# zhongzisha/multi_frame_super_resolution

Hardware: AMD Instinct MI355X
Metric: Mpix/s end-to-end (N-frame burst -> x2 SR) (higher is better)
Workload: dtype f32

## Files before the change

include/mfsr.h:

```cpp
#ifndef MFSR_H
#define MFSR_H

#include <stddef.h>
#include <stdint.h>

#ifdef __cplusplus
extern "C" {
#endif

#define MFSR_VERSION 100
#define MFSR_MAX_FUSE_GROUP 4

typedef void* mfsr_stream_t;

typedef struct { float x, y; } mfsr_float2;
typedef struct { float x, y, z; } mfsr_float3;
typedef struct { float x, y, z, w; } mfsr_float4;

typedef struct {
    const void* ptr;
    int32_t pitch;
    int32_t width;
    int32_t height;
} mfsr_tex2d;
// ... 162 lines not shown
                             int tileCount, mfsr_stream_t stream);
int mfsr_addRoundedPreShift(const mfsr_float2* preShift, int prePitch, mfsr_float2* found, int foundPitch, int countX,
                            int countY, mfsr_stream_t stream);
int mfsr_scaleFlow(mfsr_float2* flow, int pitch, int width, int height, float factor, mfsr_stream_t stream);
int mfsr_float3ToFloat4(const mfsr_float3* in, int inPitch, mfsr_float4* out, int outPitch, int width, int height,
                        mfsr_stream_t stream);
int mfsr_resampleFloat3(const mfsr_float3* in, int inPitch, int inW, int inH, mfsr_float3* out, int outPitch, int outW,
                        int outH, float u0, float u1, float v0, float v1, mfsr_stream_t stream);
int mfsr_quantize(const mfsr_float3* in, int inPitch, uint16_t* out16, uint8_t* out8, int width, int height,
                  float maxOut, mfsr_stream_t stream);
int mfsr_fill_f32(float* dst, size_t count, float value, mfsr_stream_t stream);
int mfsr_prepareFrameFused(const uint16_t* dataIn, mfsr_float3* halfOut, int halfPitch, float maxVal, int dimX, int dimY,
                           float* pyr0, int pyr0Pitch, float* pyr1, int pyr1Pitch, const float* taps, int ntaps,
                           mfsr_stream_t stream);
int mfsr_zeroRing_f32x4(mfsr_float4* img, int pitch, int width, int height, mfsr_stream_t stream);
int mfsr_set_accumulate_fast_exp(int enable);

int mfsr_trackTilesFused(const float* refImg, const float* movedImg, const mfsr_float2* preShift, int preShiftPitch,
                         mfsr_float2* coordinates, int coordinatesPitch, int imgWidth, int imgHeight, int imgPitch,
                         int maxShift, int tileSize, int tileCountX, int tileCountY, float threshold,
                         const float* refSquaredSums, mfsr_stream_t stream);
int mfsr_tileSquaredSums(const float* refImg, float* outValues, int imgWidth, int imgHeight, int imgPitch, int maxShift,
                         int tileSize, int tileCountX, int tileCountY, mfsr_stream_t stream);
int mfsr_lucasKanadeIterationFused(const mfsr_float2* shiftsIn, mfsr_float2* shiftsOut, int pitchShift,
                                   const float* refImg, const float* movedImg, int pitchImg, int width, int height,
                                   int halfWindowSize, float minDet, float outScale, mfsr_stream_t stream);
int mfsr_robustnessMaskFused(const mfsr_float3* rawImgRef, const mfsr_float3* rawImgMoved, mfsr_float4* robustnessMask,
                             mfsr_tex2d texUV, int imgWidth, int imgHeight, int imgPitch, int maskPitch, float alpha, float beta,
                             float thresholdM, mfsr_stream_t stream);
int mfsr_set_robustness_fast(int enable);
int mfsr_structureTensorFused(const float* img, int imgPitch, mfsr_float3* outImg, int outPitch, int width, int height,
                              mfsr_stream_t stream);
int mfsr_deBayerFused(const uint16_t* raw, mfsr_float3* outImage, int strideOut, int width, int height,
                      mfsr_float3 blackPoint, mfsr_float3 scale, mfsr_stream_t stream);
int mfsr_finishFused(const mfsr_float3* finalImg, const mfsr_float3* weight, int imgPitch, const mfsr_float3* fallback,
                     int fbPitch, int fbW, int fbH, float u0, float u1, float v0, float v1, mfsr_float3* outImg,
                     int outPitch, uint16_t* out16, int width, int height, float threshold, int applyGamma,
                     float maxOut, mfsr_stream_t stream);

typedef struct {
    float shiftX, shiftY;
    float rotation;
    float cosRotation, sinRotation;
    int32_t angleIndex, tx, ty, level;
    int32_t reserved[3];
} mfsr_prealign;
size_t mfsr_preAlign_pyramid_bytes(int width, int height);
size_t mfsr_preAlign_workspace_bytes(float maxAngleDeg);
int mfsr_preAlign_init(void* workspace, float maxAngleDeg, mfsr_stream_t stream);
int mfsr_preAlignPyramid(const float* img, int width, int height, int pitch, void* pyramid, mfsr_stream_t stream);
int mfsr_preAlign(const void* refPyramid, const void* movedPyramid, int width, int height, float maxAngleDeg,
                  void* workspace, mfsr_prealign* result, mfsr_stream_t stream);
int mfsr_preAlign_identity(mfsr_prealign* result, mfsr_stream_t stream);
int mfsr_trackTilesFusedBase(const float* refImg, const float* movedImg, const mfsr_float2* preShift, int preShiftPitch,
                             mfsr_float2* coordinates, int coordinatesPitch, int imgWidth, int imgHeight, int imgPitch,
// ... 249 lines not shown
```

multi_frame_super_resolution_amd/csrc/debayer.hip:

```cpp
#include <cstring>
#include "common.hpp"

static int g_cfa[4] = {MFSR_RED, MFSR_GREEN, MFSR_GREEN, MFSR_BLUE};

int mfsr_cfa_packed() { return (g_cfa[0] & 0xff) | ((g_cfa[1] & 0xff) << 8) | ((g_cfa[2] & 0xff) << 16) | ((g_cfa[3] & 0xff) << 24); }

extern "C" int mfsr_set_cfa_pattern(const int32_t pattern[4])
{
    MFSR_REQUIRE(pattern != nullptr);
    for (int i = 0; i < 4; i++) MFSR_REQUIRE(pattern[i] >= 0 && pattern[i] <= MFSR_WHITE);
    for (int i = 0; i < 4; i++) g_cfa[i] = pattern[i];
    return MFSR_OK;
}

extern "C" int mfsr_get_cfa_pattern(int32_t pattern[4])
{
    MFSR_REQUIRE(pattern != nullptr);
    for (int i = 0; i < 4; i++) pattern[i] = g_cfa[i];
    return MFSR_OK;
}

__global__ void __launch_bounds__(256) k_deBayersSubSample3(const uint16_t* __restrict__ dataIn, pix3* __restrict__ imgOut,
                                                           float maxVal, int dimX, int dimY, int strideOut, int cfa)
{
// ... 324 lines not shown
                g = RAWC(x, y, 1);
            } else if (thisPixel == MFSR_RED || thisPixel == MFSR_BLUE) {
                const int c = (thisPixel == MFSR_RED) ? 0 : 2;
                const float p = RAWC(x, y, c);
                const float xMinus2 = RAWC(x - 2, y, c), xMinus1 = RAWC(x - 1, y, 1), xPlus1 = RAWC(x + 1, y, 1),
                            xPlus2 = RAWC(x + 2, y, c);
                const float yMinus2 = RAWC(x, y - 2, c), yMinus1 = RAWC(x, y - 1, 1), yPlus1 = RAWC(x, y + 1, 1),
                            yPlus2 = RAWC(x, y + 2, c);
                const float gradientX = 0.5f * fabsf(xPlus1 - xMinus1);
                const float gradientY = 0.5f * fabsf(yPlus1 - yMinus1);
                const float laplaceX = 0.25f * fabsf(2.0f * p - xMinus2 - xPlus2);
                const float laplaceY = 0.25f * fabsf(2.0f * p - yMinus2 - yPlus2);
                const float interpolX = 0.125f * (-xMinus2 + 4.0f * xMinus1 + 2.0f * p + 4.0f * xPlus1 - xPlus2);
                const float interpolY = 0.125f * (-yMinus2 + 4.0f * yMinus1 + 2.0f * p + 4.0f * yPlus1 - yPlus2);
                const float weight = (gradientY + laplaceY) / (gradientX + gradientY + laplaceX + laplaceY + 0.000000001f);
                g = weight * interpolX + (1.0f - weight) * interpolY;
            }
#undef RAWC
        }
        s_g[ly][lx] = g;
    }
    __syncthreads();
    const int x = x0 + threadIdx.x, y = y0 + threadIdx.y;
    if (x >= width - 2 || x < 2 || y >= height - 2 || y < 2) return;
    auto GREENF = [&](int xx, int yy) { return s_g[yy - y0 + 1][xx - x0 + 1]; };
#define RAWR(xx, yy) ((RAWF(xx, yy) - L.bp[0]) * L.sc[0])
#define RAWB(xx, yy) ((RAWF(xx, yy) - L.bp[2]) * L.sc[2])
    const int thisPixel = cfa_at(cfa, y, x);
    const int thisRow = cfa_at(cfa, y, x + 1);
    const float g = GREENF(x, y);
    float r = 0.0f, b = 0.0f;
    if (thisPixel == MFSR_GREEN) {
        if (thisRow == MFSR_RED) {
            r = g + 0.5f * ((RAWR(x - 1, y) - GREENF(x - 1, y)) + (RAWR(x + 1, y) - GREENF(x + 1, y)));
            b = g + 0.5f * ((RAWB(x, y - 1) - GREENF(x, y - 1)) + (RAWB(x, y + 1) - GREENF(x, y + 1)));
        } else {
            b = g + 0.5f * ((RAWB(x - 1, y) - GREENF(x - 1, y)) + (RAWB(x + 1, y) - GREENF(x + 1, y)));
            r = g + 0.5f * ((RAWR(x, y - 1) - GREENF(x, y - 1)) + (RAWR(x, y + 1) - GREENF(x, y + 1)));
        }
    } else if (thisPixel == MFSR_RED) {
        r = RAWR(x, y);
        b = g + 0.25f * ((((RAWB(x - 1, y - 1) - GREENF(x - 1, y - 1)) + (RAWB(x + 1, y - 1) - GREENF(x + 1, y - 1))) +
                          (RAWB(x + 1, y + 1) - GREENF(x + 1, y + 1))) +
                         (RAWB(x - 1, y + 1) - GREENF(x - 1, y + 1)));
    } else if (thisPixel == MFSR_BLUE) {
        b = RAWB(x, y);
        r = g + 0.25f * ((((RAWR(x - 1, y - 1) - GREENF(x - 1, y - 1)) + (RAWR(x + 1, y - 1) - GREENF(x + 1, y - 1))) +
// ... 20 lines not shown
```

multi_frame_super_resolution_amd/csrc/glue.hip:

```cpp
#include <cmath>
#include <cstring>

#include "common.hpp"

extern "C" const char* mfsr_error_string(int code)
{
    switch (code) {
        case MFSR_OK: return "success";
        case MFSR_E_INVALID: return "invalid argument";
        case MFSR_E_UNSUPPORTED: return "unsupported parameter";
        case MFSR_E_NODEVICE: return "no HIP device";
        case MFSR_E_WORKSPACE: return "workspace too small";
        case -5: return "multi-GPU transport failed (mfsr_dist: RCCL error, or a peer of a local group failed / timed out)";
        default: break;
    }
    if (code > 0) return hipGetErrorString((hipError_t)code);
    return "unknown error";
}

extern "C" int mfsr_version(void) { return MFSR_VERSION; }

extern "C" int mfsr_device_count(void)
{
    int n = 0;
    if (hipGetDeviceCount(&n) != hipSuccess) {
        (void)hipGetLastError();
// ... 479 lines not shown
    t0 += s_t[ly][lx - 1] * 8.0f;
    t0 -= s_t[ly][lx - 2];
    t0 /= 12.0f;
    const float dx = t0;
    t0 = s_t[ly + 2][lx];
    t0 -= s_t[ly + 1][lx] * 8.0f;
    t0 += s_t[ly - 1][lx] * 8.0f;
    t0 -= s_t[ly - 2][lx];
    t0 /= 12.0f;
    const float dy = t0;
    pix3 val = {dx * dx, dy * dy, dx * dy};
    row_ptr(outImg, outPitch, y)[x] = val;
}

extern "C" int mfsr_structureTensorFused(const float* img, int imgPitch, mfsr_float3* outImg, int outPitch, int width,
                                         int height, mfsr_stream_t stream)
{
    MFSR_REQUIRE(img && outImg && width >= 4 && height >= 4 && (long long)imgPitch >= 4LL * width &&
                 (long long)outPitch >= 12LL * width && (imgPitch & 3) == 0 && (outPitch & 3) == 0);
    dim3 block(ST_TX, ST_TY), grid(mfsr_cdiv(width, ST_TX), mfsr_cdiv(height, ST_TY));
    hipLaunchKernelGGL(k_structureTensorFused, grid, block, 0, mfsr_s(stream), img, imgPitch, (pix3*)outImg, outPitch,
                       width, height);
    return mfsr_launch_status("structureTensorFused");
}

__device__ __forceinline__ float apply_weight_f(float inout, float val, float w, float threshold)
{
    if (w < threshold) {
        val += inout;
        w += 1;
    }
    inout = 0;
    if (w != 0) inout = val / w;
    return inout;
}

__device__ __forceinline__ float gamma_f(float v)
{
    if (isnan(v)) v = 0;
    v = fmaxf(fminf(v, 1.0f), 0.0f);
    if (v <= 0.0031308f) return 12.92f * v;
    return (1.0f + 0.055f) * powf(v, 1.0f / 2.4f) - 0.055f;
}

__global__ void __launch_bounds__(256)
    k_finishFused(const pix3* __restrict__ finalImg, const pix3* __restrict__ weight, int imgPitch,
// ... 147 lines not shown
```

multi_frame_super_resolution_amd/csrc/optical_flow.hip:

```cpp
#include "common.hpp"
#include "lk_math.hpp"

__global__ void __launch_bounds__(256)
    k_Warping(int width, int height, int stride, mfsr_tex2d texUV, float* __restrict__ out, mfsr_tex2d texToWarp)
{
    const int ix = threadIdx.x + blockIdx.x * blockDim.x;
    const int iy = threadIdx.y + blockIdx.y * blockDim.y;
    if (ix >= width || iy >= height) return;
    const float2 shift = tex2<ADDR_CLAMP>(texUV, ((float)ix + 0.5f) / (float)width, ((float)iy + 0.5f) / (float)height);
    const float x = ((float)ix + 0.5f + shift.x) / (float)width;
    const float y = ((float)iy + 0.5f + shift.y) / (float)height;
    row_ptr(out, stride, iy)[ix] = tex1<ADDR_MIRROR>(texToWarp, x, y);
}

extern "C" int mfsr_WarpingKernel(int width, int height, int stride, mfsr_tex2d texUV, float* out, mfsr_tex2d texToWarp,
                                  mfsr_stream_t stream)
{
    MFSR_REQUIRE(out && width > 0 && height > 0 && (long long)stride >= 4LL * width && (stride & 3) == 0);
    MFSR_REQUIRE(mfsr_tex_ok(texUV, 8) && ((uintptr_t)texUV.ptr & 7) == 0 && (texUV.pitch & 7) == 0);
    MFSR_REQUIRE(mfsr_tex_ok(texToWarp, 4) && (texToWarp.pitch & 3) == 0);
    dim3 block(64, 4), grid(mfsr_cdiv(width, 64), mfsr_cdiv(height, 4));
    hipLaunchKernelGGL(k_Warping, grid, block, 0, mfsr_s(stream), width, height, stride, texUV, out, texToWarp);
    return mfsr_launch_status("WarpingKernel");
}
// ... 57 lines not shown
    shift.x += cf * patchCenterX - sf * patchCenterY - patchCenterX;
    shift.y += sf * patchCenterX + cf * patchCenterY - patchCenterY;
    const float2 shiftPatch =
        tex2<ADDR_CLAMP>(texShift, ((float)pxX + 0.5f) / (float)imgWidth, ((float)pxY + 0.5f) / (float)imgHeight);
    shift.x += shiftPatch.x;
    shift.y += shiftPatch.y;
    row_ptr(outImg, imgPitch, pxY)[pxX] = shift;
}

extern "C" int mfsr_CreateFlowFieldFromTilesBase(mfsr_float2* outImg, mfsr_tex2d texObjShiftXY, int imgWidth, int imgHeight,
                                                 int imgPitch, const mfsr_prealign* base, mfsr_stream_t stream)
{
    MFSR_REQUIRE(outImg && base && imgWidth > 0 && imgHeight > 0);
    MFSR_REQUIRE((long long)imgPitch >= 8LL * imgWidth && (imgPitch & 7) == 0 && ((uintptr_t)outImg & 7) == 0);
    MFSR_REQUIRE(mfsr_tex_ok(texObjShiftXY, 8) && ((uintptr_t)texObjShiftXY.ptr & 7) == 0 && (texObjShiftXY.pitch & 7) == 0);
    dim3 block(64, 4), grid(mfsr_cdiv(imgWidth, 64), mfsr_cdiv(imgHeight, 4));
    hipLaunchKernelGGL(k_CreateFlowFieldFromTilesBase, grid, block, 0, mfsr_s(stream), (float2*)outImg, texObjShiftXY, imgWidth,
                       imgHeight, imgPitch, base);
    return mfsr_launch_status("CreateFlowFieldFromTilesBase");
}

__device__ __forceinline__ float deriv5(const mfsr_tex2d& t, float x, float y, float dx, float dy)
{
    float t0 = tex1<ADDR_MIRROR>(t, x + 2.0f * dx, y + 2.0f * dy);
    t0 -= tex1<ADDR_MIRROR>(t, x + 1.0f * dx, y + 1.0f * dy) * 8.0f;
    t0 += tex1<ADDR_MIRROR>(t, x - 1.0f * dx, y - 1.0f * dy) * 8.0f;
    t0 -= tex1<ADDR_MIRROR>(t, x - 2.0f * dx, y - 2.0f * dy);
    t0 /= 12.0f;
    return t0;
}

__global__ void __launch_bounds__(256) k_ComputeDerivatives(int width, int height, int stride, float* __restrict__ Ix,
                                                           float* __restrict__ Iy, float* __restrict__ Iz,
                                                           mfsr_tex2d texSource, mfsr_tex2d texTarget)
{
    const int ix = threadIdx.x + blockIdx.x * blockDim.x;
    const int iy = threadIdx.y + blockIdx.y * blockDim.y;
    if (ix >= width || iy >= height) return;
    const float dx = 1.0f / (float)width;
    const float dy = 1.0f / (float)height;
    const float x = ((float)ix + 0.5f) * dx;
    const float y = ((float)iy + 0.5f) * dy;
    float t0 = deriv5(texSource, x, y, dx, 0.0f);
    float t1 = deriv5(texTarget, x, y, dx, 0.0f);
    row_ptr(Ix, stride, iy)[ix] = (t0 + t1) * 0.5f;
    row_ptr(Iz, stride, iy)[ix] = tex1<ADDR_MIRROR>(texSource, x, y) - tex1<ADDR_MIRROR>(texTarget, x, y);
    t0 = deriv5(texSource, x, y, 0.0f, dy);
    t1 = deriv5(texTarget, x, y, 0.0f, dy);
    row_ptr(Iy, stride, iy)[ix] = (t0 + t1) * 0.5f;
}

extern "C" int mfsr_ComputeDerivativesKernel(int width, int height, int stride, float* Ix, float* Iy, float* Iz,
// ... 105 lines not shown
```

multi_frame_super_resolution_amd/csrc/pipeline.cpp:

```cpp
#include <hip/hip_runtime.h>

#include <cmath>
#include <cstdio>
#include <cstring>
#include <new>
#include <utility>
#include <vector>

#include "common.hpp"
#include "raw_stage.hpp"

namespace {

constexpr int kMaxLevels = 4;
constexpr int kMaxTimedLaunches = 4096;
constexpr int kRing = 2 * MFSR_MAX_FUSE_GROUP;
constexpr int kMaxUploadRing = 32;

inline size_t align_up(size_t v, size_t a) { return (v + a - 1) / a * a; }

struct Img {
    void* ptr = nullptr;
    int pitch = 0;
    int w = 0, h = 0;
// ... 587 lines not shown
    const int nl = ilog2(L.maxFactor) + 1;
    for (int i = 1; i < nl; i++)
        TRY(mfsr_downsample2x((const float*)pyr[i - 1].ptr, pyr[i - 1].pitch, (float*)pyr[i].ptr, pyr[i].pitch, pyr[i].w,
                              pyr[i].h, stream));
    return MFSR_OK;
}

static int set_reference_impl(mfsr_burst* b, const uint16_t* rawRef, int hrRow0, int hrRow1, mfsr_stream_t stream)
{
    MFSR_REQUIRE(b && rawRef);
    TRY(flush_pending(b, stream, false));
    const mfsr_config& c = b->cfg;
    Layout& L = b->L;
    MFSR_REQUIRE(hrRow0 >= 0 && hrRow1 > hrRow0 && hrRow1 <= L.hrH);
    MFSR_REQUIRE(!b->winNext.on || (hrRow0 == 0 && hrRow1 == L.hrH));
    b->win = b->winNext;
    if (b->win.on) {
        hrRow0 = b->win.y0;
        hrRow1 = b->win.y0 + b->win.h;
    }
    const bool whole = (hrRow0 == 0 && hrRow1 == L.hrH) || !c.fused;
    TRY(wait_uploads(b, stream));
    if (!b->refPrepared) TRY(prepare_frame(b, rawRef, L.refHalf, L.refPyr, stream));
    if (c.fused)
        for (int l = 0; l < c.levels; l++) {
            const Img& ref = L.refPyr[ilog2(c.levelFactor[l])];
            TRY(mfsr_tileSquaredSums((const float*)ref.ptr, L.refSq[l], ref.w, ref.h, ref.pitch, c.maxShift[l], c.tileSize[l],
                                     L.tcx[l], L.tcy[l], stream));
        }

    if (c.preAlign) {
        TRY(mfsr_preAlign_init(L.preWork, c.preAlignMaxAngle, stream));
        if (!b->refPrepared)
            TRY(mfsr_preAlignPyramid((const float*)L.refPyr[0].ptr, L.tw, L.th, L.refPyr[0].pitch, L.preRefPyr, stream));
    }

    static const bool refOverlap = [] {
        const char* e = getenv("MFSR_REF_OVERLAP");
        return !(e && e[0] == '0');
    }();
    mfsr_stream_t es = stream;
    b->refOnFuse = false;
    if (refOverlap && b->fuseStream && c.fused) {
        MFSR_HIP_TRY(hipEventRecord(b->evRefStart, mfsr_s(stream)));
        MFSR_HIP_TRY(hipStreamWaitEvent(b->fuseStream, b->evRefStart, 0));
        es = (mfsr_stream_t)b->fuseStream;
    }
    {
        int f0 = 0, f1 = L.th;
        if (!whole) {
            const int per = L.hrH / L.th, halo = b->ntensorTaps / 2 + 1;
            f0 = hrRow0 / per - 1 - halo;
            f1 = (hrRow1 + per - 1) / per + 1 + halo;
            f0 = f0 < 0 ? 0 : f0;
            f1 = f1 > L.th ? L.th : f1;
        }
        const int fr = f1 - f0;
        Img& ix = L.Ix;
        Img& iy = L.Iy;
        auto rows = [&](const Img& im) { return (char*)im.ptr + (size_t)f0 * im.pitch; };
        TRY(mfsr_ComputeDerivatives2Rows(L.tw, L.th, ix.pitch, (float*)ix.ptr, (float*)iy.ptr, as_tex(L.refPyr[0]), f0, fr, es));
        TRY(mfsr_ComputeStructureTensor((const float*)rows(ix), (const float*)rows(iy), (mfsr_float3*)rows(L.tensor), L.tw, fr, ix.pitch,
                                        L.tensor.pitch, es));
        TRY(mfsr_separableFilter((const float*)rows(L.tensor), L.tensor.pitch, (float*)rows(L.tensorTmp), (float*)rows(L.tensorSm),
                                 L.tensorSm.pitch, L.tw, fr, 3, b->tensorTaps, b->ntensorTaps, es));
        TRY(mfsr_ComputeKernelParam((mfsr_float3*)rows(L.tensorSm), L.tw, fr, L.tensorSm.pitch, c.Dth, c.Dtr, c.kDetail, c.kDenoise,
                                    c.kStretch, c.kShrink, es));
        TRY(mfsr_float3ToFloat4((const mfsr_float3*)rows(L.tensorSm), L.tensorSm.pitch, (mfsr_float4*)rows(L.kparam4), L.kparam4.pitch,
                                L.tw, fr, es));
    }

    const mfsr_float3 bp = {c.black[0], c.black[1], c.black[2]};
    const mfsr_float3 sc = {1.0f / c.white[0], 1.0f / c.white[1], 1.0f / c.white[2]};
    int r0 = 0, r1 = L.H;
    if (!whole) {
        r0 = (hrRow0 / c.scale - 8) & ~1;
        r1 = ((hrRow1 + c.scale - 1) / c.scale + 8 + 1) & ~1;
        r0 = r0 < 0 ? 0 : r0;
        r1 = r1 > L.H ? L.H : r1;
    }
    char* fb = (char*)L.fallback.ptr + (size_t)r0 * L.fallback.pitch;
    MFSR_HIP_TRY(hipMemsetAsync(fb, 0, (size_t)L.fallback.pitch * (r1 - r0), mfsr_s(es)));
    if (c.fused) {
        TRY(mfsr_deBayerFused(rawRef + (size_t)r0 * L.W, (mfsr_float3*)fb, L.fallback.pitch, L.W, r1 - r0, bp, sc, es));
        if (es != stream) {
            MFSR_HIP_TRY(hipEventRecord(b->evRefDone, b->fuseStream));
            b->refOnFuse = true;
        }
    } else {
        TRY(mfsr_u16ToFloat(rawRef, (float*)L.rawf.ptr, L.rawf.pitch, L.W, L.H, 1.0f, stream));
        TRY(mfsr_deBayerGreenKernel(L.W, L.H, (const float*)L.rawf.ptr, L.rawf.pitch, (mfsr_float3*)L.fallback.ptr,
                                    L.fallback.pitch, bp, sc, stream));
        TRY(mfsr_deBayerRedBlueKernel(L.W, L.H, (const float*)L.rawf.ptr, L.rawf.pitch, (mfsr_float3*)L.fallback.ptr,
                                      L.fallback.pitch, bp, sc, stream));
    }
    b->haveRef = true;
    b->refStale = false;
    b->framesSinceRef = 0;
    b->holdLastGroup = false;
    return MFSR_OK;
}

extern "C" int mfsr_burst_set_reference(mfsr_burst* b, const uint16_t* rawRef, mfsr_stream_t stream)
{
    MFSR_REQUIRE(b != nullptr);
    return set_reference_impl(b, rawRef, 0, b->L.hrH, stream);
}

extern "C" int mfsr_burst_set_reference_rows(mfsr_burst* b, const uint16_t* rawRef, int hrRow0, int hrRow1, mfsr_stream_t stream)
{
    MFSR_REQUIRE(b != nullptr);
    return set_reference_impl(b, rawRef, hrRow0, hrRow1, stream);
// ... 1845 lines not shown
```

multi_frame_super_resolution_amd/csrc/tile_tracker.hip:

```cpp
#include <cfloat>

#include <cstdlib>

#include <cstring>
#include "common.hpp"

__device__ __forceinline__ float wave_sum(float v)
{
#pragma unroll
    for (int off = 32; off >= 1; off >>= 1) v += __shfl_xor(v, off, 64);
    return v;
}
__device__ __forceinline__ float wave_max(float v)
{
#pragma unroll
    for (int off = 32; off >= 1; off >>= 1) v = fmaxf(v, __shfl_xor(v, off, 64));
    return v;
}
__device__ __forceinline__ void wave_argmin(float& v, int& idx)
{
#pragma unroll
    for (int off = 32; off >= 1; off >>= 1) {
        const float ov = __shfl_xor(v, off, 64);
        const int oi = __shfl_xor(idx, off, 64);
        const bool take = (ov < v) || (ov == v && oi < idx);
        v = take ? ov : v;
        idx = take ? oi : idx;
    }
// ... 406 lines not shown
                                                               int imgOutPitch)
{
    const int pxX = blockIdx.x * blockDim.x + threadIdx.x;
    const int pxY = blockIdx.y * blockDim.y + threadIdx.y;
    if (pxX >= imgWidth || pxY >= imgHeight) return;
    const float dx = row_ptr(imgDx, imgDxDyPitch, pxY)[pxX];
    const float dy = row_ptr(imgDy, imgDxDyPitch, pxY)[pxX];
    pix3 val = {dx * dx, dy * dy, dx * dy};
    row_ptr(outImg, imgOutPitch, pxY)[pxX] = val;
}

extern "C" int mfsr_ComputeStructureTensor(const float* imgDx, const float* imgDy, mfsr_float3* outImg, int imgWidth,
                                           int imgHeight, int imgDxDyPitch, int imgOutPitch, mfsr_stream_t stream)
{
    MFSR_REQUIRE(imgDx && imgDy && outImg && imgWidth > 0 && imgHeight > 0);
    MFSR_REQUIRE((long long)imgDxDyPitch >= 4LL * imgWidth && (long long)imgOutPitch >= 12LL * imgWidth);
    MFSR_REQUIRE((imgDxDyPitch & 3) == 0 && (imgOutPitch & 3) == 0);
    dim3 block(64, 4), grid(mfsr_cdiv(imgWidth, 64), mfsr_cdiv(imgHeight, 4));
    hipLaunchKernelGGL(k_ComputeStructureTensor, grid, block, 0, mfsr_s(stream), imgDx, imgDy, (pix3*)outImg, imgWidth,
                       imgHeight, imgDxDyPitch, imgOutPitch);
    return mfsr_launch_status("ComputeStructureTensor");
}

__device__ __forceinline__ pix3 kernel_param(pix3 grad, float Dth, float Dtr, float kDetail, float kDenoise,
                                             float kStretch, float kShrink)
{
    const float a11 = grad.x, a22 = grad.y, a12 = grad.z;
    const float help = sqrtf((a22 - a11) * (a22 - a11) + 4.0f * a12 * a12);
    float c = 2.0f * a12;
    float s = a22 - a11 + help;
    const float norm = sqrtf(c * c + s * s);
    if (norm > 0) {
        c /= norm;
        s /= norm;
    } else {
        c = 1;
        s = 0;
    }
    const float lam1 = (a11 + a22 + help) / 2.0f;
    const float lam2 = (a11 + a22 - help) / 2.0f;
    const float A = 1 + sqrtf((lam1 - lam2) * (lam1 - lam2) / ((lam1 + lam2) * (lam1 + lam2)));
    float D = 1 - sqrtf(lam1) / Dtr + Dth;
    D = fmaxf(fminf(1.0f, D), 0.0f);
    const float k1h = kDetail * kStretch * A;
    const float k2h = kDetail / kShrink * A;
    float k1 = ((1.0f - D) * k1h + D * kDetail * kDenoise);
    float k2 = ((1.0f - D) * k2h + D * kDetail * kDenoise);
    k1 *= k1;
    k2 *= k2;
    const float x2 = c, y2 = s, x1 = s, y1 = -c;
    const float b11 = k1 * x1 * x1 + x2 * x2 * k2;
    const float b12 = k1 * x1 * y1 + x2 * y2 * k2;
    const float b22 = k1 * y1 * y1 + y2 * y2 * k2;
    const float det = b11 * b22 - b12 * b12 + 0.0000000001f;
    pix3 kernel = {b22 / det, b11 / det, -b12 / det};
    return kernel;
}

__global__ void __launch_bounds__(256) k_ComputeKernelParam(pix3* __restrict__ kernelImg, int imgWidth, int imgHeight,
                                                           int imgOutPitch, float Dth, float Dtr, float kDetail,
                                                           float kDenoise, float kStretch, float kShrink)
{
    const int pxX = blockIdx.x * blockDim.x + threadIdx.x;
    const int pxY = blockIdx.y * blockDim.y + threadIdx.y;
    if (pxX >= imgWidth || pxY >= imgHeight) return;
    pix3* p = row_ptr(kernelImg, imgOutPitch, pxY) + pxX;
    *p = kernel_param(*p, Dth, Dtr, kDetail, kDenoise, kStretch, kShrink);
}

extern "C" int mfsr_ComputeKernelParam(mfsr_float3* kernelImg, int imgWidth, int imgHeight, int imgOutPitch, float Dth,
                                       float Dtr, float kDetail, float kDenoise, float kStretch, float kShrink,
                                       mfsr_stream_t stream)
{
    MFSR_REQUIRE(kernelImg && imgWidth > 0 && imgHeight > 0 && (long long)imgOutPitch >= 12LL * imgWidth);
    MFSR_REQUIRE((imgOutPitch & 3) == 0);
    dim3 block(64, 4), grid(mfsr_cdiv(imgWidth, 64), mfsr_cdiv(imgHeight, 4));
    hipLaunchKernelGGL(k_ComputeKernelParam, grid, block, 0, mfsr_s(stream), (pix3*)kernelImg, imgWidth, imgHeight,
                       imgOutPitch, Dth, Dtr, kDetail, kDenoise, kStretch, kShrink);
    return mfsr_launch_status("ComputeKernelParam");
}

// ... 476 lines not shown
        for (int y = 0; y < T; y++) box += rq[y * R];
        const float sq = refSq[min(tile0 + sl, tileCount - 1)];
        slot_dist(sl)[cand] = sq + box - 2 * cc;
    }
    __syncthreads();

    const int wave = tid >> 6, lane = tid & 63;
    if (wave < TPW && tile0 + wave < tileCount) {
        const int tileIdx = tile0 + wave;
        float minVal, maxVal;
        int minIdx;
        wave_min_argmin_max(slot_dist(wave), R * R, lane, minVal, minIdx, maxVal);
        if (lane == 0) {
            const int tileIdxY = tileIdx / tileCountX, tileIdxX = tileIdx - tileIdxY * tileCountX;
            const float2 pre = s_pre[wave];
            float2 coord = subpixel_minimum(slot_dist(wave), S, minVal, minIdx, maxVal, threshold);
            coord.x = roundf(pre.x) + coord.x;
            coord.y = roundf(pre.y) + coord.y;
            row_ptr(coordinates, coordinatesPitch, tileIdxY)[tileIdxX] = coord;
        }
    }
}

__global__ void __launch_bounds__(64)
    k_tileSquaredSums(const float* __restrict__ refImg, float* __restrict__ out, int imgWidth, int imgHeight, int imgPitch,
                      int maxShift, int tileSize, int tileCountX, int tileCountY)
{
    extern __shared__ __attribute__((aligned(16))) float s_mem[];
    const int T = tileSize, S = maxShift;
    const int tileIdx = blockIdx.x;
    const int tileIdxY = tileIdx / tileCountX, tileIdxX = tileIdx - tileIdxY * tileCountX;
    const float2 zero2 = make_float2(0.0f, 0.0f);
    for (int i = threadIdx.x; i < T * T; i += 64) {
        const int y = i / T, x = i - y * T;
        s_mem[i] = tile_fetch(refImg, imgWidth, imgHeight, imgPitch, T, tileIdxX, tileIdxY, x + S, y + S, zero2, zero2, 0.0f);
    }
    __syncthreads();
    if (threadIdx.x == 0) {
        float a = 0;
        for (int i = 0; i < T * T; i++) a += s_mem[i] * s_mem[i];
        out[tileIdx] = a;
    }
}

extern "C" int mfsr_tileSquaredSums(const float* refImg, float* outValues, int imgWidth, int imgHeight, int imgPitch,
                                    int maxShift, int tileSize, int tileCountX, int tileCountY, mfsr_stream_t stream)
{
    MFSR_REQUIRE(refImg && outValues && imgWidth > 0 && imgHeight > 0);
    MFSR_REQUIRE((long long)imgPitch >= 4LL * imgWidth && (imgPitch & 3) == 0);
    MFSR_REQUIRE(maxShift >= 1 && maxShift <= 15 && tileSize >= 4 && tileSize <= 128 && tileCountX > 0 && tileCountY > 0);
    hipLaunchKernelGGL(k_tileSquaredSums, dim3(tileCountX * tileCountY), dim3(64), sizeof(float) * tileSize * tileSize,
                       mfsr_s(stream), refImg, outValues, imgWidth, imgHeight, imgPitch, maxShift, tileSize, tileCountX,
                       tileCountY);
    return mfsr_launch_status("tileSquaredSums");
}

static int track_tiles_fused_impl(const float* refImg, const float* movedImg, const mfsr_float2* preShift, int preShiftPitch,
                                  mfsr_float2* coordinates, int coordinatesPitch, int imgWidth, int imgHeight, int imgPitch,
                                  int maxShift, int tileSize, int tileCountX, int tileCountY, float threshold,
                                  const float* refSquaredSums, const mfsr_prealign* base, float baseInvScale,
                                  const mfsr_float2* coarse, int coarsePitch, int4 up, int upOldTile, mfsr_stream_t stream,
                                  int nFrames = 1, const MfsrBatch* batch = nullptr)
{
    MfsrBatch bt;
    if (batch)
        bt = *batch;
    else
        memset(&bt, 0, sizeof(bt));
    MFSR_REQUIRE(refImg && movedImg && coordinates && imgWidth > 0 && imgHeight > 0);
    MFSR_REQUIRE((long long)imgPitch >= 4LL * imgWidth && (imgPitch & 3) == 0);
    MFSR_REQUIRE(maxShift >= 1 && maxShift <= 15 && tileSize >= 4 && tileSize <= 128 && tileCountX > 0 && tileCountY > 0);
    MFSR_REQUIRE((long long)coordinatesPitch >= 8LL * tileCountX && (coordinatesPitch & 7) == 0 &&
                 ((uintptr_t)coordinates & 7) == 0);
    if (preShift)
        MFSR_REQUIRE((long long)preShiftPitch >= 8LL * tileCountX && (preShiftPitch & 7) == 0 && ((uintptr_t)preShift & 7) == 0);
    static const bool fast = [] {
        const char* e = getenv("MFSR_TRK_FAST");
// ... 115 lines not shown
```

Before: 22350.

## Fuse kernel-parameter chain into one tiled kernel and batch squared-sum levels

Replaces the five-launch chain of derivatives, structure tensor, separable smoothing, kernel parameter and float3-to-float4 conversion with one tiled kernel. It stages the image, derivatives and horizontally filtered tensor in LDS, so the intermediates never go to global memory. It also merges the per-level tileSquaredSums launches into a single launch that indexes levels by block. The fallback memset is dropped by having the fused debayer write zeros on its border. The cost is a large LDS footprint that may limit occupancy, plus recomputing halo derivatives in every tile.

```diff
diff --git a/include/mfsr.h b/include/mfsr.h
--- a/include/mfsr.h
+++ b/include/mfsr.h
@@ -208,6 +208,12 @@
                          const float* refSquaredSums, mfsr_stream_t stream);
 int mfsr_tileSquaredSums(const float* refImg, float* outValues, int imgWidth, int imgHeight, int imgPitch, int maxShift,
                          int tileSize, int tileCountX, int tileCountY, mfsr_stream_t stream);
+typedef struct {
+    const float* refImg;
+    float* outValues;
+    int imgWidth, imgHeight, imgPitch, maxShift, tileSize, tileCountX, tileCountY, reserved;
+} mfsr_sqsum_level;
+int mfsr_tileSquaredSumsLevels(int nLevels, const mfsr_sqsum_level* levels, mfsr_stream_t stream);
 int mfsr_lucasKanadeIterationFused(const mfsr_float2* shiftsIn, mfsr_float2* shiftsOut, int pitchShift,
                                    const float* refImg, const float* movedImg, int pitchImg, int width, int height,
                                    int halfWindowSize, float minDet, float outScale, mfsr_stream_t stream);
@@ -217,6 +223,14 @@
 int mfsr_set_robustness_fast(int enable);
 int mfsr_structureTensorFused(const float* img, int imgPitch, mfsr_float3* outImg, int outPitch, int width, int height,
                               mfsr_stream_t stream);
+int mfsr_kernelParamChain(mfsr_tex2d tex, float* Ix, float* Iy, int derivPitch, mfsr_float3* tensor, mfsr_float3* tensorTmp,
+                          mfsr_float3* tensorSm, int tensorPitch, mfsr_float4* kparam4, int kparamPitch, int row0, int rows,
+                          const float* taps, int ntaps, float Dth, float Dtr, float kDetail, float kDenoise, float kStretch,
+                          float kShrink, mfsr_stream_t stream);
+int mfsr_kernelParamFused(mfsr_tex2d tex, float* Ix, float* Iy, int derivPitch, mfsr_float3* tensor, mfsr_float3* tensorTmp,
+                          mfsr_float3* tensorSm, int tensorPitch, mfsr_float4* kparam4, int kparamPitch, int row0, int rows,
+                          const float* taps, int ntaps, float Dth, float Dtr, float kDetail, float kDenoise, float kStretch,
+                          float kShrink, mfsr_stream_t stream);
 int mfsr_deBayerFused(const uint16_t* raw, mfsr_float3* outImage, int strideOut, int width, int height,
                       mfsr_float3 blackPoint, mfsr_float3 scale, mfsr_stream_t stream);
 int mfsr_finishFused(const mfsr_float3* finalImg, const mfsr_float3* weight, int imgPitch, const mfsr_float3* fallback,
diff --git a/multi_frame_super_resolution_amd/csrc/debayer.hip b/multi_frame_super_resolution_amd/csrc/debayer.hip
--- a/multi_frame_super_resolution_amd/csrc/debayer.hip
+++ b/multi_frame_super_resolution_amd/csrc/debayer.hip
@@ -370,7 +370,12 @@
     }
     __syncthreads();
     const int x = x0 + threadIdx.x, y = y0 + threadIdx.y;
-    if (x >= width - 2 || x < 2 || y >= height - 2 || y < 2) return;
+    if (x >= width || y >= height) return;
+    if (x >= width - 2 || x < 2 || y >= height - 2 || y < 2) {
+        const pix3 z = {0.0f, 0.0f, 0.0f};
+        row_ptr(outImage, strideOut, y)[x] = z;
+        return;
+    }
     auto GREENF = [&](int xx, int yy) { return s_g[yy - y0 + 1][xx - x0 + 1]; };
 #define RAWR(xx, yy) ((RAWF(xx, yy) - L.bp[0]) * L.sc[0])
 #define RAWB(xx, yy) ((RAWF(xx, yy) - L.bp[2]) * L.sc[2])
diff --git a/multi_frame_super_resolution_amd/csrc/glue.hip b/multi_frame_super_resolution_amd/csrc/glue.hip
--- a/multi_frame_super_resolution_amd/csrc/glue.hip
+++ b/multi_frame_super_resolution_amd/csrc/glue.hip
@@ -2,6 +2,7 @@
 #include <cstring>
 
 #include "common.hpp"
+#include "kernel_field.hpp"
 
 extern "C" const char* mfsr_error_string(int code)
 {
@@ -527,6 +528,155 @@
     hipLaunchKernelGGL(k_structureTensorFused, grid, block, 0, mfsr_s(stream), img, imgPitch, (pix3*)outImg, outPitch,
                        width, height);
     return mfsr_launch_status("structureTensorFused");
+}
+
+#define KPF_TX 64
+#define KPF_TY 16
+#define KPF_MAXC0 8
+struct KpfTaps {
+    float t[2 * KPF_MAXC0 + 1];
+    int n;
+};
+struct KpfShape {
+    float Dth, Dtr, kDetail, kDenoise, kStretch, kShrink;
+};
+
+__global__ void __launch_bounds__(256) k_kernelParamFused(mfsr_tex2d tex, float4* __restrict__ kparam4, int outPitch, int row0,
+                                                         int rows, KpfTaps taps, KpfShape ks)
+{
+    extern __shared__ __attribute__((aligned(16))) float s_kpf[];
+    const int c0 = taps.n / 2;
+    const int DW = KPF_TX + 2 * c0, DH = KPF_TY + 2 * c0;
+    const int SW = DW + 6, SH = DH + 6;
+    float* sImg = s_kpf;
+    float* sIx = sImg + SW * SH;
+    float* sIy = sIx + DW * DH;
+    float* sXX = sIy + DW * DH;
+    float* sYY = sXX + KPF_TX * DH;
+    float* sXY = sYY + KPF_TX * DH;
+    const int W = tex.width, H = tex.height;
+    const float* __restrict__ img = (const float*)tex.ptr;
+    const int tid = threadIdx.y * 64 + threadIdx.x;
+    const int x0 = blockIdx.x * KPF_TX, y0 = row0 + blockIdx.y * KPF_TY, yEnd = row0 + rows;
+    const int ox = x0 - c0 - 3, oy = y0 - c0 - 3;
+
+    {
+        const int stepY = 256 / SW, stepX = 256 - stepY * SW;
+        int ly = tid / SW, lx = tid - ly * SW;
+        while (ly < SH) {
+            sImg[ly * SW + lx] = row_ptr(img, tex.pitch, clampi(oy + ly, 0, H - 1))[clampi(ox + lx, 0, W - 1)];
+            lx += stepX;
+            ly += stepY;
+            if (lx >= SW) {
+                lx -= SW;
+                ly++;
+            }
+        }
+    }
+    __syncthreads();
+    {
+        auto texel = [&](int i, int j) {
+            const int li = i - ox, lj = j - oy;
+            if ((unsigned)li < (unsigned)SW && (unsigned)lj < (unsigned)SH) return sImg[lj * SW + li];
+            return row_ptr(img, tex.pitch, j)[i];
+        };
+        auto fetch = [&](float u, float v) { return tex1_with<ADDR_MIRROR>(W, H, u, v, texel); };
+        const float dx = 1.0f / (float)W;
+        const float dy = 1.0f / (float)H;
+        const int stepY = 256 / DW, stepX = 256 - stepY * DW;
+        int ly = tid / DW, lx = tid - ly * DW;
+        while (ly < DH) {
+            const int gx = clampi(x0 + lx - c0, 0, W - 1), gy = clampi(y0 + ly - c0, row0, yEnd - 1);
+            const float x = ((float)gx + 0.5f) * dx;
+            const float y = ((float)gy + 0.5f) * dy;
+            sIx[ly * DW + lx] = deriv5_with(fetch, x, y, dx, 0.0f);
+            sIy[ly * DW + lx] = deriv5_with(fetch, x, y, 0.0f, dy);
+            lx += stepX;
+            ly += stepY;
+            if (lx >= DW) {
+                lx -= DW;
+                ly++;
+            }
+        }
+    }
+    __syncthreads();
+    for (int i = tid; i < KPF_TX * DH; i += 256) {
+        const int ly = i >> 6, lx = i & 63;
+        float sxx = 0, syy = 0, sxy = 0;
+        for (int t = 0; t < taps.n; t++) {
+            const float gx = sIx[ly * DW + lx + t], gy = sIy[ly * DW + lx + t], w = taps.t[t];
+            sxx = __fadd_rn(sxx, __fmul_rn(w, __fmul_rn(gx, gx)));
+            syy = __fadd_rn(syy, __fmul_rn(w, __fmul_rn(gy, gy)));
+            sxy = __fadd_rn(sxy, __fmul_rn(w, __fmul_rn(gx, gy)));
+        }
+        sXX[i] = sxx;
+        sYY[i] = syy;
+        sXY[i] = sxy;
+    }
+    __syncthreads();
+    const int lx = threadIdx.x, gx = x0 + lx;
+#pragma unroll
+    for (int r = 0; r < KPF_TY / 4; r++) {
+        const int ly = threadIdx.y + 4 * r, gy = y0 + ly;
+        if (gx >= W || gy >= yEnd) continue;
+        pix3 s = {0.0f, 0.0f, 0.0f};
+        for (int t = 0; t < taps.n; t++) {
+            const float w = taps.t[t];
+            s.x = __fadd_rn(s.x, __fmul_rn(w, sXX[(ly + t) * KPF_TX + lx]));
+            s.y = __fadd_rn(s.y, __fmul_rn(w, sYY[(ly + t) * KPF_TX + lx]));
+            s.z = __fadd_rn(s.z, __fmul_rn(w, sXY[(ly + t) * KPF_TX + lx]));
+        }
+        const pix3 p = kernel_param(s, ks.Dth, ks.Dtr, ks.kDetail, ks.kDenoise, ks.kStretch, ks.kShrink);
+        row_ptr(kparam4, outPitch, gy)[gx] = make_float4(p.x, p.y, p.z, 0.0f);
+    }
+}
+
+extern "C" int mfsr_kernelParamChain(mfsr_tex2d tex, float* Ix, float* Iy, int derivPitch, mfsr_float3* tensor, mfsr_float3* tensorTmp,
+                                     mfsr_float3* tensorSm, int tensorPitch, mfsr_float4* kparam4, int kparamPitch, int row0, int rows,
+                                     const float* taps, int ntaps, float Dth, float Dtr, float kDetail, float kDenoise, float kStretch,
+                                     float kShrink, mfsr_stream_t stream)
+{
+    MFSR_REQUIRE(Ix && Iy && tensor && tensorTmp && tensorSm && kparam4 && mfsr_tex_ok(tex, 4));
+    MFSR_REQUIRE(row0 >= 0 && rows > 0 && row0 + rows <= tex.height);
+    const int w = tex.width;
+    auto at = [&](void* p, int pitch) { return (char*)p + (size_t)row0 * pitch; };
+    int rc = mfsr_ComputeDerivatives2Rows(w, tex.height, derivPitch, Ix, Iy, tex, row0, rows, stream);
+    if (rc) return rc;
+    rc = mfsr_ComputeStructureTensor((const float*)at(Ix, derivPitch), (const float*)at(Iy, derivPitch),
+                                     (mfsr_float3*)at(tensor, tensorPitch), w, rows, derivPitch, tensorPitch, stream);
+    if (rc) return rc;
+    rc = mfsr_separableFilter((const float*)at(tensor, tensorPitch), tensorPitch, (float*)at(tensorTmp, tensorPitch),
+                              (float*)at(tensorSm, tensorPitch), tensorPitch, w, rows, 3, taps, ntaps, stream);
+    if (rc) return rc;
+    rc = mfsr_ComputeKernelParam((mfsr_float3*)at(tensorSm, tensorPitch), w, rows, tensorPitch, Dth, Dtr, kDetail, kDenoise, kStretch,
+                                 kShrink, stream);
+    if (rc) return rc;
+    return mfsr_float3ToFloat4((const mfsr_float3*)at(tensorSm, tensorPitch), tensorPitch, (mfsr_float4*)at(kparam4, kparamPitch),
+                               kparamPitch, w, rows, stream);
+}
+
+extern "C" int mfsr_kernelParamFused(mfsr_tex2d tex, float* Ix, float* Iy, int derivPitch, mfsr_float3* tensor, mfsr_float3* tensorTmp,
+                                     mfsr_float3* tensorSm, int tensorPitch, mfsr_float4* kparam4, int kparamPitch, int row0, int rows,
+                                     const float* taps, int ntaps, float Dth, float Dtr, float kDetail, float kDenoise, float kStretch,
+                                     float kShrink, mfsr_stream_t stream)
+{
+    MFSR_REQUIRE(kparam4 && taps && mfsr_tex_ok(tex, 4) && (tex.pitch & 3) == 0);
+    MFSR_REQUIRE(ntaps > 0 && ntaps <= 99 && (ntaps & 1) == 1);
+    MFSR_REQUIRE(row0 >= 0 && rows > 0 && row0 + rows <= tex.height);
+    MFSR_REQUIRE((long long)kparamPitch >= 16LL * tex.width && (kparamPitch & 15) == 0 && ((uintptr_t)kparam4 & 15) == 0);
+    if (ntaps / 2 > KPF_MAXC0)
+        return mfsr_kernelParamChain(tex, Ix, Iy, derivPitch, tensor, tensorTmp, tensorSm, tensorPitch, kparam4, kparamPitch, row0, rows,
+                                     taps, ntaps, Dth, Dtr, kDetail, kDenoise, kStretch, kShrink, stream);
+    KpfTaps tp;
+    memset(&tp, 0, sizeof(tp));
+    memcpy(tp.t, taps, sizeof(float) * ntaps);
+    tp.n = ntaps;
+    const KpfShape ks = {Dth, Dtr, kDetail, kDenoise, kStretch, kShrink};
+    const int c0 = ntaps / 2, DW = KPF_TX + 2 * c0, DH = KPF_TY + 2 * c0;
+    const size_t lds = sizeof(float) * ((size_t)(DW + 6) * (DH + 6) + 2 * (size_t)DW * DH + 3 * (size_t)KPF_TX * DH);
+    dim3 block(64, 4), grid(mfsr_cdiv(tex.width, KPF_TX), mfsr_cdiv(rows, KPF_TY));
+    hipLaunchKernelGGL(k_kernelParamFused, grid, block, lds, mfsr_s(stream), tex, (float4*)kparam4, kparamPitch, row0, rows, tp, ks);
+    return mfsr_launch_status("kernelParamFused");
 }
 
 __device__ __forceinline__ float apply_weight_f(float inout, float val, float w, float threshold)
diff --git a/multi_frame_super_resolution_amd/csrc/kernel_field.hpp b/multi_frame_super_resolution_amd/csrc/kernel_field.hpp
--- /dev/null
+++ b/multi_frame_super_resolution_amd/csrc/kernel_field.hpp
@@ -0,0 +1,56 @@
+#pragma once
+
+#include "common.hpp"
+
+template <int MODE, typename Texel>
+__device__ __forceinline__ float tex1_with(int w, int h, float u, float v, Texel texel)
+{
+    const TexCoord c = tex_coord<MODE>(w, h, u, v);
+    return lerp4(texel(c.i0, c.j0), texel(c.i1, c.j0), texel(c.i0, c.j1), texel(c.i1, c.j1), c.a, c.b);
+}
+
+template <typename Fetch>
+__device__ __forceinline__ float deriv5_with(Fetch fetch, float x, float y, float dx, float dy)
+{
+    float t0 = fetch(x + 2.0f * dx, y + 2.0f * dy);
+    t0 -= fetch(x + 1.0f * dx, y + 1.0f * dy) * 8.0f;
+    t0 += fetch(x - 1.0f * dx, y - 1.0f * dy) * 8.0f;
+    t0 -= fetch(x - 2.0f * dx, y - 2.0f * dy);
+    t0 /= 12.0f;
+    return t0;
+}
+
+__device__ __forceinline__ pix3 kernel_param(pix3 grad, float Dth, float Dtr, float kDetail, float kDenoise,
+                                             float kStretch, float kShrink)
+{
+    const float a11 = grad.x, a22 = grad.y, a12 = grad.z;
+    const float help = sqrtf((a22 - a11) * (a22 - a11) + 4.0f * a12 * a12);
+    float c = 2.0f * a12;
+    float s = a22 - a11 + help;
+    const float norm = sqrtf(c * c + s * s);
+    if (norm > 0) {
+        c /= norm;
+        s /= norm;
+    } else {
+        c = 1;
+        s = 0;
+    }
+    const float lam1 = (a11 + a22 + help) / 2.0f;
+    const float lam2 = (a11 + a22 - help) / 2.0f;
+    const float A = 1 + sqrtf((lam1 - lam2) * (lam1 - lam2) / ((lam1 + lam2) * (lam1 + lam2)));
+    float D = 1 - sqrtf(lam1) / Dtr + Dth;
+    D = fmaxf(fminf(1.0f, D), 0.0f);
+    const float k1h = kDetail * kStretch * A;
+    const float k2h = kDetail / kShrink * A;
+    float k1 = ((1.0f - D) * k1h + D * kDetail * kDenoise);
+    float k2 = ((1.0f - D) * k2h + D * kDetail * kDenoise);
+    k1 *= k1;
+    k2 *= k2;
+    const float x2 = c, y2 = s, x1 = s, y1 = -c;
+    const float b11 = k1 * x1 * x1 + x2 * x2 * k2;
+    const float b12 = k1 * x1 * y1 + x2 * y2 * k2;
+    const float b22 = k1 * y1 * y1 + y2 * y2 * k2;
+    const float det = b11 * b22 - b12 * b12 + 0.0000000001f;
+    pix3 kernel = {b22 / det, b11 / det, -b12 / det};
+    return kernel;
+}
diff --git a/multi_frame_super_resolution_amd/csrc/optical_flow.hip b/multi_frame_super_resolution_amd/csrc/optical_flow.hip
--- a/multi_frame_super_resolution_amd/csrc/optical_flow.hip
+++ b/multi_frame_super_resolution_amd/csrc/optical_flow.hip
@@ -1,4 +1,5 @@
 #include "common.hpp"
+#include "kernel_field.hpp"
 #include "lk_math.hpp"
 
 __global__ void __launch_bounds__(256)
@@ -103,12 +104,7 @@
 
 __device__ __forceinline__ float deriv5(const mfsr_tex2d& t, float x, float y, float dx, float dy)
 {
-    float t0 = tex1<ADDR_MIRROR>(t, x + 2.0f * dx, y + 2.0f * dy);
-    t0 -= tex1<ADDR_MIRROR>(t, x + 1.0f * dx, y + 1.0f * dy) * 8.0f;
-    t0 += tex1<ADDR_MIRROR>(t, x - 1.0f * dx, y - 1.0f * dy) * 8.0f;
-    t0 -= tex1<ADDR_MIRROR>(t, x - 2.0f * dx, y - 2.0f * dy);
-    t0 /= 12.0f;
-    return t0;
+    return deriv5_with([&](float u, float v) { return tex1<ADDR_MIRROR>(t, u, v); }, x, y, dx, dy);
 }
 
 __global__ void __launch_bounds__(256) k_ComputeDerivatives(int width, int height, int stride, float* __restrict__ Ix,
diff --git a/multi_frame_super_resolution_amd/csrc/pipeline.cpp b/multi_frame_super_resolution_amd/csrc/pipeline.cpp
--- a/multi_frame_super_resolution_amd/csrc/pipeline.cpp
+++ b/multi_frame_super_resolution_amd/csrc/pipeline.cpp
@@ -633,12 +633,14 @@
     const bool whole = (hrRow0 == 0 && hrRow1 == L.hrH) || !c.fused;
     TRY(wait_uploads(b, stream));
     if (!b->refPrepared) TRY(prepare_frame(b, rawRef, L.refHalf, L.refPyr, stream));
-    if (c.fused)
+    if (c.fused) {
+        mfsr_sqsum_level lv[4];
         for (int l = 0; l < c.levels; l++) {
             const Img& ref = L.refPyr[ilog2(c.levelFactor[l])];
-            TRY(mfsr_tileSquaredSums((const float*)ref.ptr, L.refSq[l], ref.w, ref.h, ref.pitch, c.maxShift[l], c.tileSize[l],
-                                     L.tcx[l], L.tcy[l], stream));
-        }
+            lv[l] = {(const float*)ref.ptr, L.refSq[l], ref.w, ref.h, ref.pitch, c.maxShift[l], c.tileSize[l], L.tcx[l], L.tcy[l], 0};
+        }
+        TRY(mfsr_tileSquaredSumsLevels(c.levels, lv, stream));
+    }
 
     if (c.preAlign) {
         TRY(mfsr_preAlign_init(L.preWork, c.preAlignMaxAngle, stream));
@@ -667,18 +669,15 @@
             f1 = f1 > L.th ? L.th : f1;
         }
         const int fr = f1 - f0;
-        Img& ix = L.Ix;
-        Img& iy = L.Iy;
-        auto rows = [&](const Img& im) { return (char*)im.ptr + (size_t)f0 * im.pitch; };
-        TRY(mfsr_ComputeDerivatives2Rows(L.tw, L.th, ix.pitch, (float*)ix.ptr, (float*)iy.ptr, as_tex(L.refPyr[0]), f0, fr, es));
-        TRY(mfsr_ComputeStructureTensor((const float*)rows(ix), (const float*)rows(iy), (mfsr_float3*)rows(L.tensor), L.tw, fr, ix.pitch,
-                                        L.tensor.pitch, es));
-        TRY(mfsr_separableFilter((const float*)rows(L.tensor), L.tensor.pitch, (float*)rows(L.tensorTmp), (float*)rows(L.tensorSm),
-                                 L.tensorSm.pitch, L.tw, fr, 3, b->tensorTaps, b->ntensorTaps, es));
-        TRY(mfsr_ComputeKernelParam((mfsr_float3*)rows(L.tensorSm), L.tw, fr, L.tensorSm.pitch, c.Dth, c.Dtr, c.kDetail, c.kDenoise,
-                                    c.kStretch, c.kShrink, es));
-        TRY(mfsr_float3ToFloat4((const mfsr_float3*)rows(L.tensorSm), L.tensorSm.pitch, (mfsr_float4*)rows(L.kparam4), L.kparam4.pitch,
-                                L.tw, fr, es));
+        static const bool kparamFused = [] {
+            const char* e = getenv("MFSR_KPARAM_FUSED");
+            return !(e && e[0] == '0');
+        }();
+        auto field = (c.fused && kparamFused) ? mfsr_kernelParamFused : mfsr_kernelParamChain;
+        TRY(field(as_tex(L.refPyr[0]), (float*)L.Ix.ptr, (float*)L.Iy.ptr, L.Ix.pitch, (mfsr_float3*)L.tensor.ptr,
+                  (mfsr_float3*)L.tensorTmp.ptr, (mfsr_float3*)L.tensorSm.ptr, L.tensor.pitch, (mfsr_float4*)L.kparam4.ptr,
+                  L.kparam4.pitch, f0, fr, b->tensorTaps, b->ntensorTaps, c.Dth, c.Dtr, c.kDetail, c.kDenoise, c.kStretch, c.kShrink,
+                  es));
     }
 
     const mfsr_float3 bp = {c.black[0], c.black[1], c.black[2]};
@@ -691,7 +690,6 @@
         r1 = r1 > L.H ? L.H : r1;
     }
     char* fb = (char*)L.fallback.ptr + (size_t)r0 * L.fallback.pitch;
-    MFSR_HIP_TRY(hipMemsetAsync(fb, 0, (size_t)L.fallback.pitch * (r1 - r0), mfsr_s(es)));
     if (c.fused) {
         TRY(mfsr_deBayerFused(rawRef + (size_t)r0 * L.W, (mfsr_float3*)fb, L.fallback.pitch, L.W, r1 - r0, bp, sc, es));
         if (es != stream) {
@@ -699,6 +697,7 @@
             b->refOnFuse = true;
         }
     } else {
+        MFSR_HIP_TRY(hipMemsetAsync(fb, 0, (size_t)L.fallback.pitch * (r1 - r0), mfsr_s(es)));
         TRY(mfsr_u16ToFloat(rawRef, (float*)L.rawf.ptr, L.rawf.pitch, L.W, L.H, 1.0f, stream));
         TRY(mfsr_deBayerGreenKernel(L.W, L.H, (const float*)L.rawf.ptr, L.rawf.pitch, (mfsr_float3*)L.fallback.ptr,
                                     L.fallback.pitch, bp, sc, stream));
diff --git a/multi_frame_super_resolution_amd/csrc/tile_tracker.hip b/multi_frame_super_resolution_amd/csrc/tile_tracker.hip
--- a/multi_frame_super_resolution_amd/csrc/tile_tracker.hip
+++ b/multi_frame_super_resolution_amd/csrc/tile_tracker.hip
@@ -4,6 +4,7 @@
 
 #include <cstring>
 #include "common.hpp"
+#include "kernel_field.hpp"
 
 __device__ __forceinline__ float wave_sum(float v)
 {
@@ -456,41 +457,6 @@
     return mfsr_launch_status("ComputeStructureTensor");
 }
 
-__device__ __forceinline__ pix3 kernel_param(pix3 grad, float Dth, float Dtr, float kDetail, float kDenoise,
-                                             float kStretch, float kShrink)
-{
-    const float a11 = grad.x, a22 = grad.y, a12 = grad.z;
-    const float help = sqrtf((a22 - a11) * (a22 - a11) + 4.0f * a12 * a12);
-    float c = 2.0f * a12;
-    float s = a22 - a11 + help;
-    const float norm = sqrtf(c * c + s * s);
-    if (norm > 0) {
-        c /= norm;
-        s /= norm;
-    } else {
-        c = 1;
-        s = 0;
-    }
-    const float lam1 = (a11 + a22 + help) / 2.0f;
-    const float lam2 = (a11 + a22 - help) / 2.0f;
-    const float A = 1 + sqrtf((lam1 - lam2) * (lam1 - lam2) / ((lam1 + lam2) * (lam1 + lam2)));
-    float D = 1 - sqrtf(lam1) / Dtr + Dth;
-    D = fmaxf(fminf(1.0f, D), 0.0f);
-    const float k1h = kDetail * kStretch * A;
-    const float k2h = kDetail / kShrink * A;
-    float k1 = ((1.0f - D) * k1h + D * kDetail * kDenoise);
-    float k2 = ((1.0f - D) * k2h + D * kDetail * kDenoise);
-    k1 *= k1;
-    k2 *= k2;
-    const float x2 = c, y2 = s, x1 = s, y1 = -c;
-    const float b11 = k1 * x1 * x1 + x2 * x2 * k2;
-    const float b12 = k1 * x1 * y1 + x2 * y2 * k2;
-    const float b22 = k1 * y1 * y1 + y2 * y2 * k2;
-    const float det = b11 * b22 - b12 * b12 + 0.0000000001f;
-    pix3 kernel = {b22 / det, b11 / det, -b12 / det};
-    return kernel;
-}
-
 __global__ void __launch_bounds__(256) k_ComputeKernelParam(pix3* __restrict__ kernelImg, int imgWidth, int imgHeight,
                                                            int imgOutPitch, float Dth, float Dtr, float kDetail,
                                                            float kDenoise, float kStretch, float kShrink)
@@ -1013,37 +979,59 @@
     }
 }
 
-__global__ void __launch_bounds__(64)
-    k_tileSquaredSums(const float* __restrict__ refImg, float* __restrict__ out, int imgWidth, int imgHeight, int imgPitch,
-                      int maxShift, int tileSize, int tileCountX, int tileCountY)
+#define SQS_MAX_LEVELS 4
+struct SqsLevels {
+    mfsr_sqsum_level lv[SQS_MAX_LEVELS];
+    int first[SQS_MAX_LEVELS + 1];
+};
+
+__global__ void __launch_bounds__(64) k_tileSquaredSums(SqsLevels a, int nLevels)
 {
     extern __shared__ __attribute__((aligned(16))) float s_mem[];
-    const int T = tileSize, S = maxShift;
-    const int tileIdx = blockIdx.x;
-    const int tileIdxY = tileIdx / tileCountX, tileIdxX = tileIdx - tileIdxY * tileCountX;
+    int l = 0;
+    while (l + 1 < nLevels && (int)blockIdx.x >= a.first[l + 1]) l++;
+    const mfsr_sqsum_level& lv = a.lv[l];
+    const int T = lv.tileSize, S = lv.maxShift;
+    const int tileIdx = blockIdx.x - a.first[l];
+    const int tileIdxY = tileIdx / lv.tileCountX, tileIdxX = tileIdx - tileIdxY * lv.tileCountX;
     const float2 zero2 = make_float2(0.0f, 0.0f);
     for (int i = threadIdx.x; i < T * T; i += 64) {
         const int y = i / T, x = i - y * T;
-        s_mem[i] = tile_fetch(refImg, imgWidth, imgHeight, imgPitch, T, tileIdxX, tileIdxY, x + S, y + S, zero2, zero2, 0.0f);
+        s_mem[i] = tile_fetch(lv.refImg, lv.imgWidth, lv.imgHeight, lv.imgPitch, T, tileIdxX, tileIdxY, x + S, y + S, zero2, zero2, 0.0f);
     }
     __syncthreads();
     if (threadIdx.x == 0) {
-        float a = 0;
-        for (int i = 0; i < T * T; i++) a += s_mem[i] * s_mem[i];
-        out[tileIdx] = a;
-    }
+        float s = 0;
+        for (int i = 0; i < T * T; i++) s += s_mem[i] * s_mem[i];
+        lv.outValues[tileIdx] = s;
+    }
+}
+
+extern "C" int mfsr_tileSquaredSumsLevels(int nLevels, const mfsr_sqsum_level* levels, mfsr_stream_t stream)
+{
+    MFSR_REQUIRE(levels && nLevels >= 1 && nLevels <= SQS_MAX_LEVELS);
+    SqsLevels a;
+    memset(&a, 0, sizeof(a));
+    int maxT = 0;
+    for (int l = 0; l < nLevels; l++) {
+        const mfsr_sqsum_level& v = levels[l];
+        MFSR_REQUIRE(v.refImg && v.outValues && v.imgWidth > 0 && v.imgHeight > 0);
+        MFSR_REQUIRE((long long)v.imgPitch >= 4LL * v.imgWidth && (v.imgPitch & 3) == 0);
+        MFSR_REQUIRE(v.maxShift >= 1 && v.maxShift <= 15 && v.tileSize >= 4 && v.tileSize <= 128 && v.tileCountX > 0 &&
+                     v.tileCountY > 0 && (long long)v.tileCountX * v.tileCountY <= (1 << 24));
+        a.lv[l] = v;
+        a.first[l + 1] = a.first[l] + v.tileCountX * v.tileCountY;
+        maxT = v.tileSize > maxT ? v.tileSize : maxT;
+    }
+    hipLaunchKernelGGL(k_tileSquaredSums, dim3(a.first[nLevels]), dim3(64), sizeof(float) * maxT * maxT, mfsr_s(stream), a, nLevels);
+    return mfsr_launch_status("tileSquaredSums");
 }
 
 extern "C" int mfsr_tileSquaredSums(const float* refImg, float* outValues, int imgWidth, int imgHeight, int imgPitch,
                                     int maxShift, int tileSize, int tileCountX, int tileCountY, mfsr_stream_t stream)
 {
-    MFSR_REQUIRE(refImg && outValues && imgWidth > 0 && imgHeight > 0);
-    MFSR_REQUIRE((long long)imgPitch >= 4LL * imgWidth && (imgPitch & 3) == 0);
-    MFSR_REQUIRE(maxShift >= 1 && maxShift <= 15 && tileSize >= 4 && tileSize <= 128 && tileCountX > 0 && tileCountY > 0);
-    hipLaunchKernelGGL(k_tileSquaredSums, dim3(tileCountX * tileCountY), dim3(64), sizeof(float) * tileSize * tileSize,
-                       mfsr_s(stream), refImg, outValues, imgWidth, imgHeight, imgPitch, maxShift, tileSize, tileCountX,
-                       tileCountY);
-    return mfsr_launch_status("tileSquaredSums");
+    const mfsr_sqsum_level lv = {refImg, outValues, imgWidth, imgHeight, imgPitch, maxShift, tileSize, tileCountX, tileCountY, 0};
+    return mfsr_tileSquaredSumsLevels(1, &lv, stream);
 }
 
 static int track_tiles_fused_impl(const float* refImg, const float* movedImg, const mfsr_float2* preShift, int preShiftPitch,
```

After: 22530, median of 4. No clear change (+0.8%).
